# GlobalArrays/ga

Hardware: AMD Instinct MI355X
Metric: GiB/s device-resident 2-D strided f64 accumulate, 64 MiB patch; % HBM peak (higher is better)
Workload: dtype f64; 1 GPU; H; patch=2-D f64 2048x4096 patch, ld 8192 (64 MiB payload), payload_bytes=67108864, parallelism=owner-aligned x1 (no collective)

## Files before the change

### ga_amd/csrc/comex.cpp

```cpp
#include "comex_impl.hpp"
#include "../../include/ga_amd.h"
#include <hip/hip_version.h>
#include <stdio.h>
#include <stdlib.h>
#include <string.h>
#include <time.h>
#include <unistd.h>
#include <sched.h>
#include <deque>
#include <memory>
#include <algorithm>

#ifndef GAAMD_ROCM_PATH
#define GAAMD_ROCM_PATH "/opt/rocm"
#endif

namespace gaamd {

static std::vector<std::vector<int>> g_groups;

std::vector<int> group_members(int group) {
    Runtime &r = rt();
    std::vector<int> m;
    if (group == COMEX_GROUP_WORLD) {
// ... 333 lines not shown
    }

    const int64_t rb = row_bytes_of(cop, count[0]);
    int64_t slo = 0, shi = 0, dlo = 0, dhi = 0;
    side_span_host(ss, count, levels, rb, &slo, &shi);
    side_span_host(ds, count, levels, rb, &dlo, &dhi);
    View sv, dv;
    if (world == r.rank) fence_self_if_pending();
    if (world != r.rank) {
        fence_target(world);
        if (kind == X_PUT) {
            sv = local_view(src, slo, shi, false, true, hdl != nullptr);
            dv.dev = remote_view(world, dst, dlo, dhi);
            dv.hbm = segment_kind_of(world, (const char *)dst + dlo) == 1;
        } else {
            sv.dev = remote_view(world, src, slo, shi);
            sv.hbm = segment_kind_of(world, (const char *)src + slo) == 1;
            dv = local_view(dst, dlo, dhi, true, true);
        }
    } else {
        local_views(src, slo, shi, dst, dlo, dhi, sv, dv, hdl != nullptr);
    }
    if (dv.bounce) view_rows(dv, ds, count, levels, kind == X_ACC ? rb : count[0]);
    const bool bounce_only = (needs_sync(sv) || needs_sync(dv)) && !sv.staged && !dv.staged;
    const bool host_side = (needs_sync(sv) || needs_sync(dv)) && !bounce_only;
    const bool peer = kind == X_GET && world != r.rank && r.peer_src(world);
    if (peer) g_peer_gets.fetch_add(1, std::memory_order_relaxed);
    int si = 0;
    hipStream_t st;
    {
        std::lock_guard<std::mutex> g(r.launch_mu);
        stamp(1);
        if (host_side) sched_join_write(span_of(dv.dev, dlo, dhi));
        else si = sched_pick(span_of(sv.dev, slo, shi), span_of(dv.dev, dlo, dhi), payload_bytes(rb, count, levels));
        st = r.streams[si];
        stamp(2);
        int rc = launch_strided(cop, scale, sv.dev, ss, dv.dev, ds, count, levels, st, last_launch_info(), 0, ~0ull,
                                false, peer);
        stamp(3);
        if (rc == kErrPeerOrdered) rc = get_via_scratch(sv.dev, ss, dv.dev, ds, count, levels, st);
        if (rc) fatal("strided %s launch failed (code %d): misaligned elements or bad descriptor",
                      kind == X_ACC ? "acc" : (kind == X_PUT ? "put" : "get"), rc);
        if (host_side) sched_sync_all();
    }
    const bool synced = host_side || bounce_only || (!hdl && r.blocking_sync);
    if (!host_side && synced) {
        if (dv.hbm) sched_wait_flag(si);
        else GA_HIP(hipStreamSynchronize(st));
    }
    if (world != r.rank && !synced && !r.direct_pending.empty()) r.direct_pending[world] = 1;
    if (r.debug)
        fprintf(stderr, "[ga_amd %d] %s -> %d levels %d count0 %d rows %d: src %s dst %s stream %d\n", r.rank,
                kind == X_ACC ? "acc" : (kind == X_PUT ? "put" : "get"), world, levels, count[0],
                levels ? count[levels] : 1, sv.registered ? "registered" : (sv.staged ? "staged" : "device"),
                dv.registered ? "registered" : (dv.staged ? "staged" : "device"), si);
    if (host_side || bounce_only) {
        release_view(sv);
        release_view(dv);
    }
    if (hdl) {
        nb_complete_now(hdl, si, true);
        if (sv.ring) ring_commit(si, r.nb_seq[*hdl]);
    }
    stamp(4);
    return COMEX_SUCCESS;
}

// ... 124 lines not shown
        if (r.size > 1) boot_allgather(&mine_dev, devs.data(), sizeof(Dev));
        else devs[0] = mine_dev;
        r.same_dev.assign(r.size, 0);
        for (int q = 0; q < r.size; ++q)
            r.same_dev[q] = devs[q].node == r.node && !strcmp(devs[q].bus, mine_dev.bus);
        r.node_gpus = 0;
        for (int q = 0; q < r.size; ++q) {
            if (devs[q].node != r.node) continue;
            bool first = true;
            for (int k = 0; k < q && first; ++k)
                first = !(devs[k].node == r.node && !strcmp(devs[k].bus, devs[q].bus));
            if (first) ++r.node_gpus;
        }
        const char *pl = getenv("COMEX_AMD_PEER_LOADS");
        r.peer_loads = (pl && !strcmp(pl, "all")) ? 1 : ((pl && !strcmp(pl, "off")) ? 2 : 0);
        int peers = 0;
        for (int q = 0; q < r.size; ++q)
            if (r.same_node(q) && r.peer_src(q)) ++peers;
        const int pull = std::min(peers, 6);
        int sharing = 0;
        for (int q = 0; q < r.size; ++q)
            if (q != r.rank && r.same_dev[q] && !r.peer_src(q)) ++sharing;
        const char *ns = getenv("COMEX_AMD_STREAMS");
        sched_init(ns ? atoi(ns) : (sharing ? 1 : 2), pull);
        const char *op1 = getenv("COMEX_AMD_ONE_PASS");
        r.one_pass = false;
        if (!op1 || atoi(op1) != 0)
            for (int q = 0; q < r.size; ++q)
                if (q != r.rank && r.same_node(q) && !r.peer_src(q)) r.one_pass = true;
        r.own_holds = false;
    }
    const char *bs = getenv("COMEX_AMD_BLOCKING_SYNC");
    r.blocking_sync = !bs || atoi(bs) != 0;
    {
        r.direct_src = true;
        auto flag = [](const char *name) {
            const char *v = getenv(name);
            return !v || atoi(v) != 0;
        };
        r.acc_smp_direct = flag("COMEX_ENABLE_ACC_SMP");
        r.acc_self_direct = flag("COMEX_ENABLE_ACC_SELF") || r.acc_smp_direct;
        r.put_smp_direct = flag("COMEX_ENABLE_PUT_SMP");
        r.put_self_direct = flag("COMEX_ENABLE_PUT_SELF") || r.put_smp_direct;
        r.get_smp_direct = flag("COMEX_ENABLE_GET_SMP");
        r.get_self_direct = flag("COMEX_ENABLE_GET_SELF") || r.get_smp_direct;
        r.acc_packed = flag("COMEX_ENABLE_ACC_PACKED");
        r.put_packed = flag("COMEX_ENABLE_PUT_PACKED");
        r.get_packed = flag("COMEX_ENABLE_GET_PACKED");
        r.acc_iov = flag("COMEX_ENABLE_ACC_IOV");
        r.put_iov = flag("COMEX_ENABLE_PUT_IOV");
        r.get_iov = flag("COMEX_ENABLE_GET_IOV");
    }
    if (r.size > 1 || !r.acc_self_direct || !r.put_self_direct || !r.get_self_direct) {
        remote_init();
        wire_init();
    }
    r.initialized = true;
    boot_barrier();
    const char *vb = getenv("COMEX_AMD_VERBOSE");
    if (vb && atoi(vb) && r.rank == 0) {
        hipDeviceProp_t prop;
        const bool okp = hipGetDeviceProperties(&prop, r.device) == hipSuccess;
        const char *seg = getenv("COMEX_AMD_SEGMENT");
        fprintf(stderr,
                "%s: ranks %d on %d node(s), device %d (%s, %d CUs), library streams %d, "
                "staging %zu MiB/rank, segments in %s, blocking sync %d, "
// ... 58 lines not shown
    return COMEX_SUCCESS;
}

int comex_group_free(comex_group_t group) {
    if (group >= 1 && group <= (int)g_groups.size()) g_groups[group - 1].clear();
    return COMEX_SUCCESS;
}

int comex_group_rank(comex_group_t group, int *rank) {
    Runtime &r = rt();
    if (group == COMEX_GROUP_WORLD) { *rank = r.rank; return COMEX_SUCCESS; }
    const std::vector<int> &g = g_groups.at(group - 1);
    *rank = -1;
    for (int i = 0; i < (int)g.size(); ++i) if (g[i] == r.rank) *rank = i;
    return COMEX_SUCCESS;
}

int comex_group_size(comex_group_t group, int *size) {
    *size = (group == COMEX_GROUP_WORLD) ? rt().size : (int)g_groups.at(group - 1).size();
    return COMEX_SUCCESS;
}

int comex_group_translate_world(comex_group_t group, int group_rank, int *world_rank) {
    *world_rank = translate_world(group, group_rank);
    return COMEX_SUCCESS;
}

int comex_fence_proc(int proc, comex_group_t group) {
    ensure_init();
    fence_target(translate_world(group, proc));
    {
        std::lock_guard<std::mutex> g(rt().launch_mu);
        if (g_publish_conservative.load(std::memory_order_relaxed)) sched_publish_all();
        else sched_sync_all();
    }
    one_pass_reap(true);
    return COMEX_SUCCESS;
}

int comex_fence_all(comex_group_t group) {
    ensure_init();
    (void)group;
    Runtime &r = rt();
    drain_all_jobs();
    for (int t = 0; t < r.size; ++t) fence_target(t);
    {
        std::lock_guard<std::mutex> g(r.launch_mu);
        sched_sync_all();
    }
    one_pass_reap(true);
    return COMEX_SUCCESS;
}

int comex_barrier(comex_group_t group) {
    ensure_init();
    comex_fence_all(group);
    if (group == COMEX_GROUP_WORLD) boot_barrier();
    else members_barrier(group_members(group), group);
    return COMEX_SUCCESS;
}

int comex_put(void *src, void *dst, int bytes, int proc, comex_group_t group) {
    return xfer_contig(X_PUT, 0, nullptr, src, dst, bytes, proc, group, nullptr);
}
int comex_puts(void *src, int *src_stride, void *dst, int *dst_stride, int *count, int stride_levels, int proc,
               comex_group_t group) {
    return xfer(X_PUT, 0, nullptr, src, src_stride, dst, dst_stride, count, stride_levels, proc, group, nullptr);
}
int comex_putv(comex_giov_t *darr, int len, int proc, comex_group_t group) {
    return xfer_vec(X_PUT, 0, nullptr, darr, len, proc, group, nullptr);
}
int comex_nbput(void *src, void *dst, int bytes, int proc, comex_group_t group, comex_request_t *h) {
    return xfer_contig(X_PUT, 0, nullptr, src, dst, bytes, proc, group, h);
}
int comex_nbputs(void *src, int *src_stride, void *dst, int *dst_stride, int *count, int stride_levels, int proc,
                 comex_group_t group, comex_request_t *h) {
    return xfer(X_PUT, 0, nullptr, src, src_stride, dst, dst_stride, count, stride_levels, proc, group, h);
}
int comex_nbputv(comex_giov_t *darr, int len, int proc, comex_group_t group, comex_request_t *h) {
    return xfer_vec(X_PUT, 0, nullptr, darr, len, proc, group, h);
}
// ... 66 lines not shown
    if (g_nb_job[*h]) {
        progress_jobs();
        if (job_pending(g_nb_job[*h])) { *status = 1; return COMEX_SUCCESS; }
        g_nb_job[*h] = 0;
    }
    if (g_nb_rseq[*h]) {
        if (r.shm->done[r.li(r.rank)][r.li(g_nb_rt[*h])].load(std::memory_order_acquire) < g_nb_rseq[*h]) {
            *status = 1;
            return COMEX_SUCCESS;
        }
        g_nb_rseq[*h] = 0;
    }
    if (!sched_complete(r.nb_stream[*h], r.nb_seq[*h], false)) { *status = 1; return COMEX_SUCCESS; }
    r.nb_used[*h] = false;
    *h = -1;
    return COMEX_SUCCESS;
}

int comex_wait_all(comex_group_t group) {
    stamp(5);
    ensure_init();
    (void)group;
    Runtime &r = rt();
    drain_all_jobs();
    for (int t = 0; t < (int)g_direct_last.size(); ++t)
        if (g_direct_last[t]) wait_done(t, g_direct_last[t]);
    for (int i = 0; i < kMaxNb; ++i) {
        g_nb_job[i] = 0;
        g_nb_rseq[i] = 0;
    }
    {
        std::lock_guard<std::mutex> g(r.launch_mu);
        stamp(6);
        sched_sync_all();
        stamp(7);
    }
    one_pass_reap(true);
    for (int i = 0; i < kMaxNb; ++i) r.nb_used[i] = false;
    return COMEX_SUCCESS;
}

int comex_wait_proc(int proc, comex_group_t group) {
    (void)proc;
    return comex_wait_all(group);
}

int comex_rmw(int op, void *ploc, void *prem, int extra, int proc, comex_group_t group) {
    ensure_init();
    Runtime &r = rt();
    progress_jobs();
    const int world = translate_world(group, proc);
    int bytes, swap;
    uint64_t val;
    switch (op) {
    case COMEX_FETCH_AND_ADD: bytes = 4; swap = 0; val = (uint64_t)(uint32_t)extra; break;
    case COMEX_FETCH_AND_ADD_LONG: bytes = 8; swap = 0; val = (uint64_t)(int64_t)extra; break;
    case COMEX_SWAP: { int v; memcpy(&v, ploc, 4); bytes = 4; swap = 1; val = (uint64_t)(uint32_t)v; break; }
    case COMEX_SWAP_LONG: { int64_t v; memcpy(&v, ploc, 8); bytes = 8; swap = 1; val = (uint64_t)v; break; }
    default: fatal("comex_rmw: unknown op %d", op);
    }
    if (!ploc || !prem) fatal("comex_rmw: NULL ploc or prem");
    uint64_t old = 0;
    if (world == r.rank) {
        fence_self_if_pending();
        old = rmw_local(swap, prem, bytes, val);
    } else if (!r.same_node(world)) {
        check_remote(world, prem, 0, bytes);
// ... 109 lines not shown
int gaamd_diag(const char *key, long long value, unsigned long long *out, int nout) {
    if (!key) return -1;
    if (!strcmp(key, "stamps")) {
        if (out && nout >= 8)
            for (int k = 0; k < 8; ++k) out[k] = g_stamp[k];
        if (value >= 0) {
            if (value) memset(g_stamp, 0, sizeof(g_stamp));
            g_stamp_on.store(value != 0, std::memory_order_relaxed);
        }
        return 0;
    }
    if (!strcmp(key, "stale_gen")) {
        g_diag_stale_gen.store(value);
        return 0;
    }
    if (!strcmp(key, "stale_granule")) {
        g_diag_stale_granule.store(value);
        return 0;
    }
    if (!strcmp(key, "host_range")) {
        if (!out || nout < 2) return -1;
        out[0] = host_cpu_range_probe(out[0], out[1], value != 0) ? 1 : 0;
        return 0;
    }
    if (!strcmp(key, "publish")) {
        if (out && nout >= 1) out[0] = g_publish_conservative.load() ? 1 : 0;
        if (value >= 0) g_publish_conservative.store(value != 0);
        return 0;
    }
    if (!strcmp(key, "drop_chunk")) {
        g_diag_drop_chunk.store(value);
        return 0;
    }
    if (!strcmp(key, "peer_gets")) {
        if (out && nout >= 1) out[0] = g_peer_gets.load(std::memory_order_relaxed);
        return 0;
    }
    if (!strcmp(key, "vmm_window")) {
        if (!out || nout < 2) return -1;
        vmm_window_usage(&out[0], &out[1]);
        return 0;
    }
    if (!strcmp(key, "pinned_threads")) {
        if (out && nout >= 1) out[0] = views_pinned_threads();
        return 0;
    }
    if (!strcmp(key, "iov_host_sides")) {
        if (out && nout >= 1) out[0] = g_iov_host_sides.load(std::memory_order_relaxed);
        return 0;
    }
    return -1;
}

int gaamd_iov_path_counts(unsigned long long counts[4]) {
    for (int k = 0; k < 4; ++k) counts[k] = g_iov_path[k].load(std::memory_order_relaxed);
    return 0;
}

int gaamd_toggle_counts(unsigned long long counts[3]) {
    for (int k = 0; k < 3; ++k) counts[k] = g_toggle[k].load(std::memory_order_relaxed);
    return 0;
}

int gaamd_route_counts(unsigned long long counts[4]) {
    for (int k = 0; k < 4; ++k) counts[k] = g_route[k].load(std::memory_order_relaxed);
    return 0;
// ... 8 lines not shown
```

### ga_amd/csrc/plumbing.hip

```cpp
#include "gaamd_kernels.h"
#include "runtime.hpp"
#include <string.h>
#include <stdlib.h>
#include <dlfcn.h>

namespace gaamd {

LaunchInfo g_last;
LaunchInfo *last_launch_info() { return &g_last; }

static hipStream_t stream_of(void *s) {
    if (s) return (hipStream_t)s;
    Runtime &r = rt();
    if (r.stream) return r.stream;
    return nullptr;
}

__device__ __forceinline__ uint64_t splitmix64_at(uint64_t seed, uint64_t i) {
    uint64_t z = seed + (i + 1) * 0x9E3779B97F4A7C15ULL;
    z = (z ^ (z >> 30)) * 0xBF58476D1CE4E5B9ULL;
    z = (z ^ (z >> 27)) * 0x94D049BB133111EBULL;
    return z ^ (z >> 31);
}

__global__ __launch_bounds__(256) void k_fill(void *dst, long n, int type, uint64_t seed) {
    for (long i = (long)blockIdx.x * blockDim.x + threadIdx.x; i < n; i += (long)gridDim.x * blockDim.x) {
        const uint64_t x = splitmix64_at(seed, (uint64_t)i);
        switch (type) {
        case 0: ((double *)dst)[i] = ((double)(x >> 11) * 0x1.0p-53) * 2.0 - 1.0; break;
        case 1: ((float *)dst)[i] = ((float)(x >> 40) * 0x1.0p-24f) * 2.0f - 1.0f; break;
        case 2: ((int32_t *)dst)[i] = (int32_t)(x >> 43) - (1 << 20); break;
        default: ((int64_t *)dst)[i] = (int64_t)(x >> 43) - (1 << 20); break;
        }
    }
}

__global__ __launch_bounds__(256) void k_fill_word(uint64_t *dst, long n, uint64_t word) {
    for (long i = (long)blockIdx.x * blockDim.x + threadIdx.x; i < n; i += (long)gridDim.x * blockDim.x) dst[i] = word;
}

}

using namespace gaamd;

extern "C" {

int gaamd_strided(int op, const void *scale, const void *src, const int *src_stride, void *dst,
                  const int *dst_stride, const int *count, int stride_levels, void *stream) {
// ... 160 lines not shown
int gaamd_set_tuning(const char *key, int value) {
    if (!strcmp(key, "streams")) {
        Runtime &r = rt();
        if (!r.initialized || value < 1 || value > 8) return -1;
        std::lock_guard<std::mutex> g(r.launch_mu);
        const int old = (int)r.streams.size();
        sched_resize(value);
        return old;
    }
    int *f = tuning_field(key);
    if (!f) return -1;
    if (!strcmp(key, "block") && value != 0 && value != 64 && value != 128) return -1;
    const int old = *f;
    *f = value;
    return old;
}

int gaamd_get_tuning(const char *key) {
    if (!strcmp(key, "streams")) return (int)rt().streams.size();
    int *f = tuning_field(key);
    return f ? *f : -1;
}

int gaamd_device_count(void) {
    int n = 0;
    if (hipGetDeviceCount(&n) != hipSuccess) {
        (void)hipGetLastError();
        return 0;
    }
    return n;
}

int gaamd_set_device(int dev) { return hipSetDevice(dev) == hipSuccess ? 0 : -1; }
void *gaamd_stream(void) { return rt().stream; }
void *gaamd_stream_at(int i) {
    Runtime &r = rt();
    return (i >= 0 && i < (int)r.streams.size()) ? (void *)r.streams[i] : nullptr;
}

void *gaamd_dev_malloc(size_t bytes) {
    void *p = nullptr;
    if (hipMalloc(&p, bytes) != hipSuccess) {
        (void)hipGetLastError();
        segment_cache_flush();
        if (hipMalloc(&p, bytes) != hipSuccess) return nullptr;
    }
    addr_event('a', p, bytes, -1);
    return p;
}
int gaamd_dev_free(void *p) {
    hipDeviceptr_t base = nullptr;
    size_t size = 0;
    if (hipMemGetAddressRange(&base, &size, (hipDeviceptr_t)p) == hipSuccess) addr_event('f', p, size, -1);
    else (void)hipGetLastError();
    return hipFree(p) == hipSuccess ? 0 : -1;
}

void *gaamd_host_malloc(size_t bytes) {
    void *p = nullptr;
    if (hipHostMalloc(&p, bytes, hipHostMallocMapped | hipHostMallocPortable) != hipSuccess) return nullptr;
    return p;
}
int gaamd_host_free(void *p) { return hipHostFree(p) == hipSuccess ? 0 : -1; }

int gaamd_memcpy(void *dst, const void *src, size_t bytes) {
    return hipMemcpy(dst, src, bytes, hipMemcpyDefault) == hipSuccess ? 0 : -1;
}
int gaamd_memcpy2d(void *dst, size_t dpitch, const void *src, size_t spitch, size_t width, size_t height) {
    return hipMemcpy2D(dst, dpitch, src, spitch, width, height, hipMemcpyDefault) == hipSuccess ? 0 : -1;
}
int gaamd_memset(void *dst, int value, size_t bytes) {
    return hipMemset(dst, value, bytes) == hipSuccess ? 0 : -1;
}
int gaamd_sync(void *stream) {
    Runtime &r = rt();
    if (!stream && r.initialized) {
        std::lock_guard<std::mutex> g(r.launch_mu);
        sched_sync_all();
        return 0;
    }
    hipStream_t s = stream_of(stream);
    hipError_t e = s ? hipStreamSynchronize(s) : hipDeviceSynchronize();
    return e == hipSuccess ? 0 : -(int)e;
}

int gaamd_join(void) {
    Runtime &r = rt();
    if (!r.initialized) return -1;
    std::lock_guard<std::mutex> g(r.launch_mu);
    sched_join();
    return 0;
}

int gaamd_num_streams(void) { return (int)rt().streams.size(); }

int gaamd_fill_word(void *dst, long n, unsigned long long word, void *stream) {
    if (n <= 0) return 0;
    if ((uintptr_t)dst & 7) return -2;
    long blocks = (n + 255) / 256;
    if (blocks > 65536) blocks = 65536;
    hipLaunchKernelGGL(k_fill_word, dim3((unsigned)blocks), dim3(256), 0, stream_of(stream), (uint64_t *)dst, n,
                       (uint64_t)word);
    return hipGetLastError() == hipSuccess ? 0 : -1;
}

int gaamd_fill(void *dst, long n, int type, unsigned long long seed, void *stream) {
    if (n <= 0) return 0;
    if (type < 0 || type > 3) return -2;
    long blocks = (n + 255) / 256;
    if (blocks > 65536) blocks = 65536;
    hipLaunchKernelGGL(k_fill, dim3((unsigned)blocks), dim3(256), 0, stream_of(stream), dst, n, type,
                       (uint64_t)seed);
    return hipGetLastError() == hipSuccess ? 0 : -1;
}
// ... 35 lines not shown
```

### ga_amd/csrc/remote.cpp

```cpp
#include "comex_impl.hpp"
#include <stdio.h>
#include <stdlib.h>
#include <string.h>
#include <unistd.h>
#include <sched.h>
#include <time.h>
#include <algorithm>
#include <deque>
#include <mutex>
#include <thread>

namespace gaamd {

constexpr unsigned kOwnerEventFlags = hipEventDisableTiming | hipEventReleaseToSystem;

static const char *peer_staging_or_die(int src) {
    const char *p = rt().peer_staging[src];
    if (!p) fatal("rank %d's staging buffer is not mapped here (IPC open failed at comex_init)", src);
    return p;
}

std::vector<std::deque<Pending>> g_pend;

uint64_t sub_ring_bytes() {
// ... 524 lines not shown
            if (!published && g_publish_conservative.load(std::memory_order_relaxed)) {
                std::lock_guard<std::mutex> g(r.launch_mu);
                sched_publish_all();
                published = true;
            }
            RJob *j = find_job(c.job);
            post_request(t, j->op, j->scale, (uint64_t)(uintptr_t)j->dst, j->ds, j->count, j->levels,
                         (uint64_t)t * sub + c.off, c.len, c.rb, c.re);
            --j->outstanding;
            g_chunk_ev.push_back(c.ev);
            o.pop_front();
            any = true;
        }
    }
    for (RJob &j : g_jobs) {
        while (j.next_i < j.nchunks) {
            const uint64_t c = (j.first + j.next_i) % j.nchunks;
            const uint64_t rb = c * j.per_req, re = std::min(j.rows, rb + j.per_req);
            const uint64_t len = (re - rb) * (uint64_t)j.count[0];
            uint64_t off = 0;
            if (!try_stage_alloc(j.t, ring_len(len), off)) break;
            const uint64_t seq = ++r.posted[j.t];
            g_pend[j.t].push_back({seq, off, ring_len(len)});
            r.stage_head[j.t] = off + ring_len(len);
            char *stage = r.staging + (size_t)j.t * sub + off;
            hipEvent_t ev;
            if (g_chunk_ev.empty())
                GA_HIP(hipEventCreateWithFlags(&ev, hipEventDisableTiming | hipEventReleaseToSystem));
            else { ev = g_chunk_ev.back(); g_chunk_ev.pop_back(); }
            {
                std::lock_guard<std::mutex> g(r.launch_mu);
                const int si = j.staged_src ? 0 : sched_pick(span_of(j.sv.dev, j.slo, j.shi),
                                                             span_of(stage, 0, (int64_t)len), len);
                const int rc = launch_strided(kOpCopy, nullptr, j.sv.dev, j.ss, stage - (int64_t)rb * j.count[0],
                                              j.pstride, j.count, j.levels, r.streams[si], nullptr, rb, re);
                if (rc) fatal("pack launch failed (%d)", rc);
                GA_HIP(hipEventRecord(ev, r.streams[si]));
            }
            g_out[j.t].push_back({j.id, off, len, rb, re, ev});
            ++j.outstanding;
            ++j.next_i;
            any = true;
        }
    }
    for (auto it = g_jobs.begin(); it != g_jobs.end();) {
        if (it->next_i >= it->nchunks && it->outstanding == 0) {
            release_view(it->sv);
            it = g_jobs.erase(it);
            any = true;
        } else {
            ++it;
        }
    }
    return any;
}

static void backoff(unsigned &spins) {
    if (++spins > 256) sched_yield();
}

void run_job(int id) {
    for (unsigned spins = 0; find_job(id); backoff(spins))
        if (progress_jobs()) spins = 0;
}

bool target_busy(int t) {
// ... 173 lines not shown
```

### ga_amd/csrc/runtime.hpp

```cpp
#pragma once
#include <stdint.h>
#include <stddef.h>
#include <atomic>
#include <vector>
#include <mutex>
#include <thread>
#include <hip/hip_runtime_api.h>
#include "../../include/ga_amd.h"

namespace gaamd {

[[noreturn]] void fatal(const char *fmt, ...);
void trace(int level, const char *fmt, ...) __attribute__((format(printf, 2, 3)));

#define GA_HIP(call)                                                                  \
    do {                                                                              \
        hipError_t e_ = (call);                                                       \
        if (e_ != hipSuccess)                                                         \
            ::gaamd::fatal("%s failed: %s (%s:%d)", #call, hipGetErrorString(e_),     \
                           __FILE__, __LINE__);                                       \
    } while (0)

#define GA_ASSERT(cond, msg)                                                          \
    do {                                                                              \
// ... 74 lines not shown
struct VmmBlock {
    char *va = nullptr;
    size_t bytes = 0;
    hipMemGenericAllocationHandle_t handle{};
    int fd = -1;
    bool imported = false;
};

struct Segment {
    bool live = false;
    bool vmm = false;
    VmmBlock vmm_local;
    std::vector<VmmBlock> vmm_peer;
    bool device = true;
    void *local = nullptr;
    size_t local_bytes = 0;
    bool exported = false;
    hipIpcMemHandle_t handle;
    std::vector<PeerMap> peer;
};

struct Runtime {
    bool initialized = false;
    bool boot_ready = false;
    int rank = 0, size = 1, local_rank = 0, device = 0;
    int nnodes = 1, node = 0, node_size = 1;
    std::vector<int> node_of;
    std::vector<int> node_index;
    int li(int q) const { return node_index.empty() ? q : node_index[q]; }
    bool same_node(int q) const { return node_of.empty() || node_of[q] == node; }
    hipStream_t stream = nullptr;
    std::vector<hipStream_t> streams;
    bool blocking_sync = true;
    bool acc_self_direct = true, acc_smp_direct = true, put_self_direct = true, put_smp_direct = true;
    bool get_self_direct = true, get_smp_direct = true;
    bool acc_packed = true, put_packed = true, get_packed = true;
    bool acc_iov = true, put_iov = true, get_iov = true;
    bool direct_src = true;
    int debug = 0;
    gaamd_allgather_fn ag = nullptr;
    gaamd_barrier_fn bar = nullptr;
    void *ctx = nullptr;
    bool hooks = false;
    NodeShm *shm = nullptr;
    size_t shm_bytes = 0;
    std::vector<Segment> segs;
    std::mutex seg_mu;
    int nb_stream[kMaxNb] = {};
    uint64_t nb_seq[kMaxNb] = {};
    bool nb_used[kMaxNb] = {};
    int nb_next = 0;
    char *staging = nullptr;
    size_t staging_bytes = 0;
    std::vector<char *> peer_staging;
    std::vector<uint64_t> posted;
    std::vector<uint64_t> stage_head;
    std::vector<uint8_t> direct_pending;
    std::thread progress;
    std::atomic<bool> stop{false};
    std::mutex launch_mu;
    std::vector<uint8_t> same_dev;
    int node_gpus = 1;
    int peer_loads = 0;
    bool peer_src(int q) const {
        if (q == rank || peer_loads == 2) return false;
        return peer_loads == 1 || q >= (int)same_dev.size() || !same_dev[q];
    }
    int user_streams = 2;
    bool one_pass = false;
    bool own_holds = false;
};

Runtime &rt();

void boot_init();
void boot_allgather(const void *send, void *recv, size_t bytes);
void boot_barrier();
void boot_finalize();

void segment_cache_flush();
void sched_init(int nstreams, int pull_streams = 0);
void sched_fini();
void sched_resize(int nstreams);
void own_write_guard(const Span &dst);
int sched_pick(const Span &src, const Span &dst, uint64_t payload = 0, int prefer = -1);
void sched_join();
void sched_wait_flag(int s);
void sched_flag_init();
void sched_flag_fini();
void sched_join_write(const Span &dst);
void sched_sync_all();
void sched_publish_all();
extern std::atomic<bool> g_publish_conservative;
uint64_t sched_track(int s);
bool sched_complete(int s, uint64_t seq, bool wait);
uint64_t sched_epoch();

void wire_init();
void wire_finalize();
void wire_detach();
bool wire_active();
void wire_send_strided(int op, const void *scale, const char *src_dev, const int *ss, uint64_t dst,
                       const int *ds, const int *count, int levels, int t);
void wire_get_strided(uint64_t src, const int *ss, char *dst_dev, const int *ds, const int *count, int levels,
                      int t);
void wire_send_iov(int op, const void *scale, const uint64_t *src_dev, const uint64_t *dst, int n, int bytes,
                   bool serial, int t);
void wire_get_iov(const uint64_t *src, const uint64_t *dst_dev, int n, int bytes, int t);
void wire_fence(int t);
void msg_send(int to, int tag, const void *buf, size_t len);
size_t msg_recv(int from, int tag, void *buf, size_t buflen, int *src);
uint64_t wire_rmw(int t, int swap, uint64_t addr, int bytes, uint64_t val);
bool wire_lock(int t, int mutex, bool acquire);
uint64_t rmw_local(int swap, void *addr, int bytes, uint64_t val);
bool mutex_try_local(int owner, int mutex);
void mutex_release_local(int owner, int mutex);
bool segment_of_rank(int owner, uint64_t p, int64_t lo, int64_t hi);
bool segment_local(const void *p, int64_t lo, int64_t hi);
int segment_kind(const void *p);
void addr_event(char kind, const void *p, size_t bytes, int peer);
// ... 10 lines not shown
```

### ga_amd/csrc/sched.cpp

```cpp
#include <atomic>
#include "runtime.hpp"
#include "gaamd_kernels.h"
#include <string.h>
#include <stdlib.h>
#include <deque>
#include <algorithm>

namespace gaamd {

namespace {
constexpr int kHist = 64;
struct Entry {
    int stream;
    Span src, dst;
};
std::vector<Entry> g_hist;
std::vector<hipEvent_t> g_ev;
int g_rr = 0;
int g_base = -1;
unsigned g_base_waited = 0;

inline bool overlap(const Span &a, const Span &b) { return a.lo < b.hi && b.lo < a.hi && a.lo < a.hi && b.lo < b.hi; }

constexpr uint64_t kMarkEvery = 16;
struct Mark {
    uint64_t seq;
    hipEvent_t ev;
};
struct Marks {
    uint64_t issued = 0, done = 0, marked = 0;
    std::deque<Mark> q;
};
std::vector<Marks> g_marks;
std::vector<hipEvent_t> g_mark_pool;
std::mutex g_marks_mu;

void marks_reset_done() {
    for (Marks &m : g_marks) {
        m.done = m.marked = m.issued;
        for (const Mark &k : m.q) g_mark_pool.push_back(k.ev);
        m.q.clear();
    }
}

void mark_now(int s) {
    Marks &m = g_marks[s];
    if (m.marked == m.issued) return;
    hipEvent_t e;
    if (g_mark_pool.empty()) GA_HIP(hipEventCreateWithFlags(&e, hipEventDisableTiming));
    else { e = g_mark_pool.back(); g_mark_pool.pop_back(); }
    GA_HIP(hipEventRecord(e, rt().streams[s]));
    m.q.push_back({m.issued, e});
    m.marked = m.issued;
}
}

uint64_t sched_track(int s) {
    std::lock_guard<std::mutex> g(g_marks_mu);
    if (s < 0 || s >= (int)g_marks.size()) return 0;
    Marks &m = g_marks[s];
    const uint64_t seq = ++m.issued;
    if (seq - m.marked >= kMarkEvery) mark_now(s);
    return seq;
}

bool sched_complete(int s, uint64_t seq, bool wait) {
    std::unique_lock<std::mutex> g(g_marks_mu);
    if (seq == 0 || s < 0 || s >= (int)g_marks.size()) return true;
    Marks &m = g_marks[s];
    if (seq <= m.done) return true;
    if (m.marked < seq) mark_now(s);
    while (!m.q.empty()) {
        const Mark k = m.q.front();
        hipError_t e = hipEventQuery(k.ev);
        if (e == hipErrorNotReady && wait) {
            g.unlock();
            e = hipEventSynchronize(k.ev);
            g.lock();
            if (m.q.empty() || m.q.front().ev != k.ev) {
                if (m.done >= seq) return true;
                continue;
            }
        }
        if (e == hipErrorNotReady) return false;
        if (e != hipSuccess) fatal("operation failed: %s", hipGetErrorString(e));
        m.done = k.seq;
        g_mark_pool.push_back(k.ev);
        m.q.pop_front();
        if (m.done >= seq) return true;
    }
    return m.done >= seq;
}

static std::atomic<uint64_t> g_epoch{0};
uint64_t sched_epoch() { return g_epoch.load(std::memory_order_relaxed); }

void sched_init(int n, int pull) {
    Runtime &r = rt();
    g_epoch.fetch_add(1, std::memory_order_relaxed);
    if (n < 1) n = 1;
    if (n > 8) n = 8;
    if (pull < 0) pull = 0;
    if (pull > 8) pull = 8;
    r.user_streams = n;
    n += pull;
    r.streams.assign(1, r.stream);
    for (int i = 1; i < n; ++i) {
        hipStream_t s;
        GA_HIP(hipStreamCreateWithFlags(&s, hipStreamDefault));
        r.streams.push_back(s);
    }
    g_ev.assign(n, nullptr);
    for (int i = 0; i < n; ++i) GA_HIP(hipEventCreateWithFlags(&g_ev[i], hipEventDisableTiming));
    std::lock_guard<std::mutex> g(g_marks_mu);
    g_marks.assign(n, Marks());
    g_hist.clear();
    g_rr = 0;
    g_base = -1;
    sched_flag_init();
}

void sched_resize(int n) {
    Runtime &r = rt();
    const int pull = (int)r.streams.size() - r.user_streams;
    sched_sync_all();
    sched_fini();
    r.streams.clear();
    sched_init(n, pull);
}

static std::vector<hipEvent_t> g_pub_ev;
std::atomic<bool> g_publish_conservative{false};

void sched_fini() {
    Runtime &r = rt();
    for (hipEvent_t e : g_pub_ev) (void)hipEventDestroy(e);
    g_pub_ev.clear();
    for (size_t i = 1; i < r.streams.size(); ++i) (void)hipStreamDestroy(r.streams[i]);
    for (hipEvent_t e : g_ev) (void)hipEventDestroy(e);
    g_ev.clear();
    std::lock_guard<std::mutex> g(g_marks_mu);
    marks_reset_done();
    for (hipEvent_t e : g_mark_pool) (void)hipEventDestroy(e);
    g_mark_pool.clear();
    g_marks.clear();
    r.streams.clear();
    g_hist.clear();
}

static void wait_on(int waiter, int producer) {
    Runtime &r = rt();
    GA_HIP(hipEventRecord(g_ev[producer], r.streams[producer]));
    GA_HIP(hipStreamWaitEvent(r.streams[waiter], g_ev[producer], 0));
}

void sched_join() {
    Runtime &r = rt();
    const int n = (int)r.streams.size();
    if (n > 1) {
        for (int x = 1; x < n; ++x) wait_on(0, x);
        for (int x = 1; x < n; ++x) wait_on(x, 0);
    }
    g_hist.clear();
    g_base = -1;
}

void sched_join_write(const Span &dst) {
    own_write_guard(dst);
    sched_join();
}

void sched_sync_all() {
    Runtime &r = rt();
    for (hipStream_t s : r.streams) GA_HIP(hipStreamSynchronize(s));
    for (uint8_t &p : r.direct_pending) p = 0;
    {
        std::lock_guard<std::mutex> g(g_marks_mu);
        marks_reset_done();
    }
    g_hist.clear();
    g_base = -1;
}

void sched_publish_all() {
    Runtime &r = rt();
    while (g_pub_ev.size() < r.streams.size()) {
        hipEvent_t e;
        GA_HIP(hipEventCreateWithFlags(&e, hipEventDisableTiming | hipEventReleaseToSystem));
        g_pub_ev.push_back(e);
    }
    for (size_t i = 0; i < r.streams.size(); ++i) GA_HIP(hipEventRecord(g_pub_ev[i], r.streams[i]));
    sched_sync_all();
}

namespace {
uint64_t *g_flag_host = nullptr, *g_flag_dev = nullptr;
std::vector<uint64_t> g_flag_seq;
}

void sched_flag_init() {
    if (g_flag_host) return;
    GA_HIP(hipHostMalloc((void **)&g_flag_host, 64 * sizeof(uint64_t), hipHostMallocMapped | hipHostMallocCoherent));
    GA_HIP(hipHostGetDevicePointer((void **)&g_flag_dev, g_flag_host, 0));
    memset(g_flag_host, 0, 64 * sizeof(uint64_t));
    g_flag_seq.assign(64, 0);
    const int rc = launch_flag(g_flag_dev + 63, 0, rt().stream);
    if (rc) fatal("completion flag launch failed (%d)", rc);
    GA_HIP(hipStreamSynchronize(rt().stream));
}

void sched_wait_flag(int s) {
    Runtime &r = rt();
    uint64_t v;
    volatile uint64_t *f;
    {
        std::lock_guard<std::mutex> g(r.launch_mu);
        sched_flag_init();
        if (s < 0 || s >= 64) fatal("stream index %d out of range", s);
        v = ++g_flag_seq[s];
        const int rc = launch_flag(g_flag_dev + s, v, r.streams[s]);
        if (rc) fatal("completion flag launch failed (%d)", rc);
        f = g_flag_host + s;
    }
    for (unsigned long spins = 0; __atomic_load_n(f, __ATOMIC_ACQUIRE) < v; ++spins) {
        if ((spins & 0xfffff) == 0xfffff) {
            const hipError_t e = hipStreamQuery(r.streams[s]);
            if (e == hipSuccess) break;
            if (e != hipErrorNotReady) fatal("stream failed: %s", hipGetErrorString(e));
        }
        __builtin_ia32_pause();
    }
}

void sched_flag_fini() {
    if (g_flag_host) (void)hipHostFree(g_flag_host);
    g_flag_host = g_flag_dev = nullptr;
    g_flag_seq.clear();
}

constexpr uint64_t kBigPayload = 192ull << 20;
constexpr uint64_t kSmallPayload = 8ull << 20;

int sched_pick(const Span &src, const Span &dst, uint64_t payload, int prefer) {
    Runtime &r = rt();
    own_write_guard(dst);
    const int n = (int)r.streams.size();
    if (n <= 1) return 0;
    const int nu = std::max(1, std::min(r.user_streams, n));
    if ((int)g_hist.size() >= kHist) {
        const int s0 = g_hist.front().stream;
        bool one = g_base < 0 || g_base == s0;
        for (const Entry &e : g_hist) one = one && e.stream == s0;
        if (one) {
            g_hist.clear();
            if (g_base != s0) g_base_waited = 1u << s0;
            g_base = s0;
        } else {
            sched_join();
        }
    }
    unsigned mask = 0;
    int last = -1;
    for (const Entry &e : g_hist) {
        if (overlap(dst, e.dst) || overlap(dst, e.src) || overlap(src, e.dst)) {
            mask |= 1u << e.stream;
            last = e.stream;
        }
    }
    int s;
    if (!mask) {
        if (prefer >= 0 && prefer < n) {
            s = prefer;
        } else {
            if (payload == 0 || (payload >= kSmallPayload && payload < kBigPayload)) g_rr = (g_rr + 1) % nu;
            s = g_rr % nu;
        }
    } else {
        s = last;
        for (int x = 0; x < n; ++x)
            if (x != s && (mask & (1u << x))) wait_on(s, x);
    }
    if (g_base >= 0 && !(g_base_waited & (1u << s))) {
        wait_on(s, g_base);
        g_base_waited |= 1u << s;
        if (g_base_waited == (1u << n) - 1) g_base = -1;
    }
    g_hist.push_back({s, src, dst});
    return s;
}

}
```

### ga_amd/csrc/views.cpp

```cpp
#include "comex_impl.hpp"
#include <string.h>
#include <sys/syscall.h>
#include <unistd.h>
#include <algorithm>
#include <deque>
#include <mutex>
#include <vector>

namespace gaamd {

bool direct_view(void *p, char **dev, bool *hbm) {
    if (hbm) *hbm = false;
    if (const int k = segment_kind(p)) {
        *dev = (char *)p;
        if (hbm) *hbm = k == 1;
        return true;
    }
    hipPointerAttribute_t at;
    memset(&at, 0, sizeof(at));
    hipError_t e = hipPointerGetAttributes(&at, p);
    if (e == hipSuccess && (at.type == hipMemoryTypeDevice || at.type == hipMemoryTypeManaged)) {
        *dev = (char *)p;
        if (hbm) *hbm = at.type == hipMemoryTypeDevice;
        return true;
// ... 171 lines not shown
    if (g.q.empty()) g.head = 0;
    const int64_t mis = (int64_t)(((uintptr_t)p + lo) % kRingAlign);
    const int64_t need = (mis + n + kRingAlign - 1) / kRingAlign * kRingAlign;
    int64_t off = g.head;
    if (off + need > kRingBytes) off = 0;
    while (ring_busy(g, off, off + need)) ring_retire(g);
    if (g.q.empty()) g.head = off;
    g.pend_off = off;
    g.pend_end = off + need;
    g.head = off + need;
    memcpy(g.host + off + mis, (char *)p + lo, (size_t)n);
    v.host = (char *)p;
    v.lo = lo;
    v.hi = hi;
    v.ring = true;
    v.dev = g.dev + off + mis - lo;
    return true;
}

void ring_commit(int stream, uint64_t seq) {
    NbRing &g = pins().ring;
    if (g.pend_off < 0) return;
    g.q.push_back({g.pend_off, g.pend_end, stream, seq, sched_epoch()});
    g.pend_off = -1;
}

static void stage_view(View &v, void *p, int64_t lo, int64_t hi, bool is_dst) {
    Runtime &r = rt();
    v.host = (char *)p;
    v.lo = lo;
    v.hi = hi;
    GA_HIP(hipMalloc((void **)&v.staged, (size_t)(hi - lo)));
    GA_HIP(hipMemcpyAsync(v.staged, (char *)p + lo, (size_t)(hi - lo), hipMemcpyHostToDevice, r.stream));
    v.dev = v.staged - lo;
    v.copy_back = is_dst;
}

void local_views(void *src, int64_t slo, int64_t shi, void *dst, int64_t dlo, int64_t dhi,
                        View &sv, View &dv, bool ring_src) {
    char *d = nullptr;
    const bool sd = direct_view(src, &d, &sv.hbm);
    if (sd) sv.dev = d;
    const bool dd = direct_view(dst, &d, &dv.hbm);
    if (dd) dv.dev = d;
    uintptr_t s0 = 0, s1 = 0, d0 = 0, d1 = 0;
    if (!sd) page_range(src, slo, shi, s0, s1);
    if (!dd) page_range(dst, dlo, dhi, d0, d1);
    if (!sd && !dd && s0 < d1 && d0 < s1) {
        const uintptr_t b0 = std::min((uintptr_t)src + slo, (uintptr_t)dst + dlo);
        const uintptr_t b1 = std::max((uintptr_t)src + shi, (uintptr_t)dst + dhi);
        if ((int64_t)(b1 - b0) <= kBounceMax) {
            bounce_view(dv, (void *)b0, 0, (int64_t)(b1 - b0), true, 1);
            char *base = dv.dev;
            sv.dev = base + ((uintptr_t)src - b0);
            dv.dev = base + ((uintptr_t)dst - b0);
            dv.host = (char *)dst;
            dv.lo = dlo;
            dv.hi = dhi;
            dv.wb_host = (char *)dst;
            dv.wb_bounce = dv.bounce + ((uintptr_t)dst - b0);
            return;
        }
        const uintptr_t u0 = std::min(s0, d0), u1 = std::max(s1, d1);
        char *base = nullptr;
        if (register_range(u0, u1, &base)) {
            sv.registered = (void *)u0;
// ... 62 lines not shown
```

Baseline: 6063 GiB/s.

## Complete fences and waits via device flag spin instead of stream synchronize

Adds per-stream enqueue/sync logs and uses a device-written completion flag with host spin-polling in wait_all, fence, and single-op completion paths. Only streams with outstanding work are waited on, and streams with work that needs the runtime (copies, external use) still fall back to hipStreamSynchronize. This is meant to avoid the latency of blocking runtime synchronization on every wait or fence. It adds bookkeeping on each launch and spins a host core while waiting.

New measurement: 6020 GiB/s. Within noise of the previous version (-0.7%).

```diff
diff --git a/ga_amd/csrc/comex.cpp b/ga_amd/csrc/comex.cpp
--- a/ga_amd/csrc/comex.cpp
+++ b/ga_amd/csrc/comex.cpp
@@ -389,7 +389,8 @@
         std::lock_guard<std::mutex> g(r.launch_mu);
         stamp(1);
         if (host_side) sched_join_write(span_of(dv.dev, dlo, dhi));
-        else si = sched_pick(span_of(sv.dev, slo, shi), span_of(dv.dev, dlo, dhi), payload_bytes(rb, count, levels));
+        else si = sched_pick(span_of(sv.dev, slo, shi), span_of(dv.dev, dlo, dhi), payload_bytes(rb, count, levels), -1,
+                             dv.hbm);
         st = r.streams[si];
         stamp(2);
         int rc = launch_strided(cop, scale, sv.dev, ss, dv.dev, ds, count, levels, st, last_launch_info(), 0, ~0ull,
@@ -580,6 +581,8 @@
     }
     const char *bs = getenv("COMEX_AMD_BLOCKING_SYNC");
     r.blocking_sync = !bs || atoi(bs) != 0;
+    const char *fw = getenv("COMEX_AMD_FLAG_WAIT");
+    r.flag_wait = !fw || atoi(fw) != 0;
     {
         r.direct_src = true;
         auto flag = [](const char *name) {
@@ -704,7 +707,7 @@
     {
         std::lock_guard<std::mutex> g(rt().launch_mu);
         if (g_publish_conservative.load(std::memory_order_relaxed)) sched_publish_all();
-        else sched_sync_all();
+        else sched_complete_all(kWaitFence);
     }
     one_pass_reap(true);
     return COMEX_SUCCESS;
@@ -718,7 +721,7 @@
     for (int t = 0; t < r.size; ++t) fence_target(t);
     {
         std::lock_guard<std::mutex> g(r.launch_mu);
-        sched_sync_all();
+        sched_complete_all(kWaitFence);
     }
     one_pass_reap(true);
     return COMEX_SUCCESS;
@@ -851,7 +854,7 @@
     {
         std::lock_guard<std::mutex> g(r.launch_mu);
         stamp(6);
-        sched_sync_all();
+        sched_complete_all(kWaitAll);
         stamp(7);
     }
     one_pass_reap(true);
@@ -1027,6 +1030,10 @@
         g_diag_drop_chunk.store(value);
         return 0;
     }
+    if (!strcmp(key, "wait_paths")) {
+        sched_wait_counts(out, nout, value == 1);
+        return 0;
+    }
     if (!strcmp(key, "peer_gets")) {
         if (out && nout >= 1) out[0] = g_peer_gets.load(std::memory_order_relaxed);
         return 0;
diff --git a/ga_amd/csrc/plumbing.hip b/ga_amd/csrc/plumbing.hip
--- a/ga_amd/csrc/plumbing.hip
+++ b/ga_amd/csrc/plumbing.hip
@@ -10,10 +10,10 @@
 LaunchInfo *last_launch_info() { return &g_last; }
 
 static hipStream_t stream_of(void *s) {
-    if (s) return (hipStream_t)s;
-    Runtime &r = rt();
-    if (r.stream) return r.stream;
-    return nullptr;
+    Runtime &r = rt();
+    hipStream_t st = s ? (hipStream_t)s : r.stream;
+    if (st && r.initialized) sched_note_stream(st);
+    return st;
 }
 
 __device__ __forceinline__ uint64_t splitmix64_at(uint64_t seed, uint64_t i) {
@@ -240,10 +240,16 @@
 }
 
 int gaamd_set_device(int dev) { return hipSetDevice(dev) == hipSuccess ? 0 : -1; }
-void *gaamd_stream(void) { return rt().stream; }
+void *gaamd_stream(void) {
+    Runtime &r = rt();
+    if (r.initialized) sched_note(0, false);
+    return r.stream;
+}
 void *gaamd_stream_at(int i) {
     Runtime &r = rt();
-    return (i >= 0 && i < (int)r.streams.size()) ? (void *)r.streams[i] : nullptr;
+    if (i < 0 || i >= (int)r.streams.size()) return nullptr;
+    sched_note(i, false);
+    return (void *)r.streams[i];
 }
 
 void *gaamd_dev_malloc(size_t bytes) {
@@ -287,7 +293,7 @@
         sched_sync_all();
         return 0;
     }
-    hipStream_t s = stream_of(stream);
+    hipStream_t s = stream ? (hipStream_t)stream : r.stream;
     hipError_t e = s ? hipStreamSynchronize(s) : hipDeviceSynchronize();
     return e == hipSuccess ? 0 : -(int)e;
 }
diff --git a/ga_amd/csrc/remote.cpp b/ga_amd/csrc/remote.cpp
--- a/ga_amd/csrc/remote.cpp
+++ b/ga_amd/csrc/remote.cpp
@@ -580,6 +580,7 @@
                 std::lock_guard<std::mutex> g(r.launch_mu);
                 const int si = j.staged_src ? 0 : sched_pick(span_of(j.sv.dev, j.slo, j.shi),
                                                              span_of(stage, 0, (int64_t)len), len);
+                if (j.staged_src) sched_note(0, false);
                 const int rc = launch_strided(kOpCopy, nullptr, j.sv.dev, j.ss, stage - (int64_t)rb * j.count[0],
                                               j.pstride, j.count, j.levels, r.streams[si], nullptr, rb, re);
                 if (rc) fatal("pack launch failed (%d)", rc);
diff --git a/ga_amd/csrc/runtime.hpp b/ga_amd/csrc/runtime.hpp
--- a/ga_amd/csrc/runtime.hpp
+++ b/ga_amd/csrc/runtime.hpp
@@ -130,6 +130,7 @@
     hipStream_t stream = nullptr;
     std::vector<hipStream_t> streams;
     bool blocking_sync = true;
+    bool flag_wait = true;
     bool acc_self_direct = true, acc_smp_direct = true, put_self_direct = true, put_smp_direct = true;
     bool get_self_direct = true, get_smp_direct = true;
     bool acc_packed = true, put_packed = true, get_packed = true;
@@ -181,9 +182,14 @@
 void sched_fini();
 void sched_resize(int nstreams);
 void own_write_guard(const Span &dst);
-int sched_pick(const Span &src, const Span &dst, uint64_t payload = 0, int prefer = -1);
+int sched_pick(const Span &src, const Span &dst, uint64_t payload = 0, int prefer = -1, bool hbm_only = false);
 void sched_join();
+void sched_note(int s, bool hbm_only);
+void sched_note_stream(hipStream_t st);
 void sched_wait_flag(int s);
+enum WaitKind { kWaitAll = 0, kWaitOne, kWaitFence, kWaitBlocking, kWaitOther, kWaitKinds };
+void sched_complete_all(int kind);
+void sched_wait_counts(unsigned long long *out, int nout, bool reset);
 void sched_flag_init();
 void sched_flag_fini();
 void sched_join_write(const Span &dst);
diff --git a/ga_amd/csrc/sched.cpp b/ga_amd/csrc/sched.cpp
--- a/ga_amd/csrc/sched.cpp
+++ b/ga_amd/csrc/sched.cpp
@@ -21,6 +21,20 @@
 unsigned g_base_waited = 0;
 
 inline bool overlap(const Span &a, const Span &b) { return a.lo < b.hi && b.lo < a.hi && a.lo < a.hi && b.lo < b.hi; }
+
+constexpr int kMaxStreams = 16;
+struct StreamLog {
+    std::atomic<uint64_t> enq{0}, rt{0}, synced{0};
+};
+StreamLog g_log[kMaxStreams];
+std::atomic<unsigned long long> g_wait_count[kWaitKinds][2];
+
+inline void raise(std::atomic<uint64_t> &a, uint64_t v) {
+    uint64_t cur = a.load(std::memory_order_relaxed);
+    while (cur < v && !a.compare_exchange_weak(cur, v, std::memory_order_relaxed)) {}
+}
+inline bool log_outstanding(int s) { return g_log[s].enq.load(std::memory_order_relaxed) > g_log[s].synced.load(std::memory_order_relaxed); }
+inline bool log_needs_runtime(int s) { return g_log[s].rt.load(std::memory_order_relaxed) > g_log[s].synced.load(std::memory_order_relaxed); }
 
 constexpr uint64_t kMarkEvery = 16;
 struct Mark {
@@ -55,6 +69,27 @@
 }
 }
 
+void sched_note(int s, bool hbm_only) {
+    if (s < 0 || s >= kMaxStreams) return;
+    const uint64_t e = g_log[s].enq.fetch_add(1, std::memory_order_relaxed) + 1;
+    if (!hbm_only) raise(g_log[s].rt, e);
+}
+
+void sched_note_stream(hipStream_t st) {
+    Runtime &r = rt();
+    const int n = std::min((int)r.streams.size(), kMaxStreams);
+    for (int s = 0; s < n; ++s)
+        if (r.streams[s] == st) sched_note(s, false);
+}
+
+void sched_wait_counts(unsigned long long *out, int nout, bool reset) {
+    for (int k = 0; k < kWaitKinds; ++k)
+        for (int j = 0; j < 2; ++j) {
+            const unsigned long long v = reset ? g_wait_count[k][j].exchange(0) : g_wait_count[k][j].load();
+            if (out && 2 * k + j < nout) out[2 * k + j] = v;
+        }
+}
+
 uint64_t sched_track(int s) {
     std::lock_guard<std::mutex> g(g_marks_mu);
     if (s < 0 || s >= (int)g_marks.size()) return 0;
@@ -64,11 +99,22 @@
     return seq;
 }
 
+static bool flag_complete_stream(int s);
+
 bool sched_complete(int s, uint64_t seq, bool wait) {
+    if (wait && seq && rt().flag_wait) {
+        bool open;
+        {
+            std::lock_guard<std::mutex> g(g_marks_mu);
+            open = s >= 0 && s < (int)g_marks.size() && seq > g_marks[s].done;
+        }
+        if (open && flag_complete_stream(s)) return true;
+    }
     std::unique_lock<std::mutex> g(g_marks_mu);
     if (seq == 0 || s < 0 || s >= (int)g_marks.size()) return true;
     Marks &m = g_marks[s];
     if (seq <= m.done) return true;
+    if (wait) g_wait_count[kWaitOne][1].fetch_add(1, std::memory_order_relaxed);
     if (m.marked < seq) mark_now(s);
     while (!m.q.empty()) {
         const Mark k = m.q.front();
@@ -84,7 +130,7 @@
         }
         if (e == hipErrorNotReady) return false;
         if (e != hipSuccess) fatal("operation failed: %s", hipGetErrorString(e));
-        m.done = k.seq;
+        m.done = std::max(m.done, k.seq);
         g_mark_pool.push_back(k.ev);
         m.q.pop_front();
         if (m.done >= seq) return true;
@@ -112,6 +158,11 @@
     }
     g_ev.assign(n, nullptr);
     for (int i = 0; i < n; ++i) GA_HIP(hipEventCreateWithFlags(&g_ev[i], hipEventDisableTiming));
+    for (StreamLog &l : g_log) {
+        l.enq.store(0, std::memory_order_relaxed);
+        l.rt.store(0, std::memory_order_relaxed);
+        l.synced.store(0, std::memory_order_relaxed);
+    }
     std::lock_guard<std::mutex> g(g_marks_mu);
     g_marks.assign(n, Marks());
     g_hist.clear();
@@ -154,7 +205,7 @@
     GA_HIP(hipStreamWaitEvent(r.streams[waiter], g_ev[producer], 0));
 }
 
-void sched_join() {
+static void join_streams() {
     Runtime &r = rt();
     const int n = (int)r.streams.size();
     if (n > 1) {
@@ -165,14 +216,18 @@
     g_base = -1;
 }
 
+void sched_join() {
+    join_streams();
+    sched_note(0, false);
+}
+
 void sched_join_write(const Span &dst) {
     own_write_guard(dst);
     sched_join();
 }
 
-void sched_sync_all() {
-    Runtime &r = rt();
-    for (hipStream_t s : r.streams) GA_HIP(hipStreamSynchronize(s));
+static void all_streams_done() {
+    Runtime &r = rt();
     for (uint8_t &p : r.direct_pending) p = 0;
     {
         std::lock_guard<std::mutex> g(g_marks_mu);
@@ -181,6 +236,19 @@
     g_hist.clear();
     g_base = -1;
 }
+
+static void sync_all_streams(int kind) {
+    Runtime &r = rt();
+    const int n = (int)r.streams.size();
+    uint64_t upto[kMaxStreams];
+    for (int s = 0; s < n && s < kMaxStreams; ++s) upto[s] = g_log[s].enq.load(std::memory_order_relaxed);
+    for (hipStream_t s : r.streams) GA_HIP(hipStreamSynchronize(s));
+    for (int s = 0; s < n && s < kMaxStreams; ++s) raise(g_log[s].synced, upto[s]);
+    g_wait_count[kind][1].fetch_add((unsigned long long)n, std::memory_order_relaxed);
+    all_streams_done();
+}
+
+void sched_sync_all() { sync_all_streams(kWaitOther); }
 
 void sched_publish_all() {
     Runtime &r = rt();
@@ -209,27 +277,124 @@
     GA_HIP(hipStreamSynchronize(rt().stream));
 }
 
+namespace {
+struct FlagWait {
+    unsigned mask = 0;
+    uint64_t value[kMaxStreams], upto[kMaxStreams];
+};
+
+void flag_launch(FlagWait &w, int s) {
+    Runtime &r = rt();
+    sched_flag_init();
+    if (s < 0 || s >= kMaxStreams || s >= (int)r.streams.size()) fatal("stream index %d out of range", s);
+    w.upto[s] = g_log[s].enq.load(std::memory_order_relaxed);
+    w.value[s] = ++g_flag_seq[s];
+    const int rc = launch_flag(g_flag_dev + s, w.value[s], r.streams[s]);
+    if (rc) fatal("completion flag launch failed (%d)", rc);
+    w.mask |= 1u << s;
+}
+
+void flag_spin(const FlagWait &w) {
+    Runtime &r = rt();
+    unsigned left = w.mask;
+    for (unsigned long spins = 0; left; ++spins) {
+        for (int s = 0; s < kMaxStreams; ++s)
+            if ((left >> s & 1u) && __atomic_load_n(g_flag_host + s, __ATOMIC_ACQUIRE) >= w.value[s]) left &= ~(1u << s);
+        if (!left) break;
+        if ((spins & 0xfffff) == 0xfffff) {
+            for (int s = 0; s < kMaxStreams; ++s) {
+                if (!(left >> s & 1u)) continue;
+                const hipError_t e = hipStreamQuery(r.streams[s]);
+                if (e == hipSuccess) left &= ~(1u << s);
+                else if (e != hipErrorNotReady) fatal("stream failed: %s", hipGetErrorString(e));
+            }
+        }
+        __builtin_ia32_pause();
+    }
+}
+}
+
 void sched_wait_flag(int s) {
     Runtime &r = rt();
-    uint64_t v;
-    volatile uint64_t *f;
+    if (!r.flag_wait) {
+        GA_HIP(hipStreamSynchronize(r.streams[s]));
+        g_wait_count[kWaitBlocking][1].fetch_add(1, std::memory_order_relaxed);
+        return;
+    }
+    FlagWait w;
+    bool clean;
     {
         std::lock_guard<std::mutex> g(r.launch_mu);
-        sched_flag_init();
-        if (s < 0 || s >= 64) fatal("stream index %d out of range", s);
-        v = ++g_flag_seq[s];
-        const int rc = launch_flag(g_flag_dev + s, v, r.streams[s]);
-        if (rc) fatal("completion flag launch failed (%d)", rc);
-        f = g_flag_host + s;
-    }
-    for (unsigned long spins = 0; __atomic_load_n(f, __ATOMIC_ACQUIRE) < v; ++spins) {
-        if ((spins & 0xfffff) == 0xfffff) {
-            const hipError_t e = hipStreamQuery(r.streams[s]);
-            if (e == hipSuccess) break;
-            if (e != hipErrorNotReady) fatal("stream failed: %s", hipGetErrorString(e));
-        }
-        __builtin_ia32_pause();
-    }
+        flag_launch(w, s);
+        clean = !log_needs_runtime(s);
+    }
+    flag_spin(w);
+    if (clean) raise(g_log[s].synced, w.upto[s]);
+    g_wait_count[kWaitBlocking][0].fetch_add(1, std::memory_order_relaxed);
+}
+
+static bool flag_complete_stream(int s) {
+    Runtime &r = rt();
+    FlagWait w;
+    uint64_t issued;
+    {
+        std::lock_guard<std::mutex> g(r.launch_mu);
+        if (s < 0 || s >= kMaxStreams || s >= (int)r.streams.size() || log_needs_runtime(s)) return false;
+        {
+            std::lock_guard<std::mutex> gm(g_marks_mu);
+            if (s >= (int)g_marks.size()) return false;
+            issued = g_marks[s].issued;
+        }
+        if (log_outstanding(s)) flag_launch(w, s);
+    }
+    if (w.mask) {
+        flag_spin(w);
+        raise(g_log[s].synced, w.upto[s]);
+        g_wait_count[kWaitOne][0].fetch_add(1, std::memory_order_relaxed);
+    }
+    std::lock_guard<std::mutex> gm(g_marks_mu);
+    if (s >= (int)g_marks.size()) return true;
+    Marks &m = g_marks[s];
+    m.done = std::max(m.done, issued);
+    while (!m.q.empty() && m.q.front().seq <= m.done && hipEventQuery(m.q.front().ev) == hipSuccess) {
+        g_mark_pool.push_back(m.q.front().ev);
+        m.q.pop_front();
+    }
+    return true;
+}
+
+void sched_complete_all(int kind) {
+    Runtime &r = rt();
+    if (!r.flag_wait) {
+        sync_all_streams(kind);
+        return;
+    }
+    const int n = std::min((int)r.streams.size(), kMaxStreams);
+    FlagWait w;
+    unsigned runtime = 0;
+    uint64_t upto[kMaxStreams];
+    for (int s = 0; s < n; ++s) {
+        if (!log_outstanding(s)) continue;
+        if (log_needs_runtime(s)) {
+            runtime |= 1u << s;
+            upto[s] = g_log[s].enq.load(std::memory_order_relaxed);
+        } else {
+            flag_launch(w, s);
+        }
+    }
+    for (int s = 0; s < n; ++s) {
+        if (!(runtime >> s & 1u)) continue;
+        GA_HIP(hipStreamSynchronize(r.streams[s]));
+        raise(g_log[s].synced, upto[s]);
+        g_wait_count[kind][1].fetch_add(1, std::memory_order_relaxed);
+    }
+    flag_spin(w);
+    for (int s = 0; s < n; ++s) {
+        if (!(w.mask >> s & 1u)) continue;
+        raise(g_log[s].synced, w.upto[s]);
+        g_wait_count[kind][0].fetch_add(1, std::memory_order_relaxed);
+    }
+    all_streams_done();
 }
 
 void sched_flag_fini() {
@@ -241,11 +406,14 @@
 constexpr uint64_t kBigPayload = 192ull << 20;
 constexpr uint64_t kSmallPayload = 8ull << 20;
 
-int sched_pick(const Span &src, const Span &dst, uint64_t payload, int prefer) {
+int sched_pick(const Span &src, const Span &dst, uint64_t payload, int prefer, bool hbm_only) {
     Runtime &r = rt();
     own_write_guard(dst);
     const int n = (int)r.streams.size();
-    if (n <= 1) return 0;
+    if (n <= 1) {
+        sched_note(0, hbm_only);
+        return 0;
+    }
     const int nu = std::max(1, std::min(r.user_streams, n));
     if ((int)g_hist.size() >= kHist) {
         const int s0 = g_hist.front().stream;
@@ -256,7 +424,7 @@
             if (g_base != s0) g_base_waited = 1u << s0;
             g_base = s0;
         } else {
-            sched_join();
+            join_streams();
         }
     }
     unsigned mask = 0;
@@ -286,6 +454,7 @@
         if (g_base_waited == (1u << n) - 1) g_base = -1;
     }
     g_hist.push_back({s, src, dst});
+    sched_note(s, hbm_only);
     return s;
 }
 
diff --git a/ga_amd/csrc/views.cpp b/ga_amd/csrc/views.cpp
--- a/ga_amd/csrc/views.cpp
+++ b/ga_amd/csrc/views.cpp
@@ -227,6 +227,7 @@
     v.hi = hi;
     GA_HIP(hipMalloc((void **)&v.staged, (size_t)(hi - lo)));
     GA_HIP(hipMemcpyAsync(v.staged, (char *)p + lo, (size_t)(hi - lo), hipMemcpyHostToDevice, r.stream));
+    sched_note(0, false);
     v.dev = v.staged - lo;
     v.copy_back = is_dst;
 }
```
